# ori-drs/gpmp2

Measured on AMD Instinct MI355X. Metric: trajectories/sec, higher is better.
Workload: dtype f64; 1 GPU; WAMFactorGraphExample: 7-DOF WAM, 100 steps x 5 GP-interp, 200^3 SDF (Synth200), 64 random-init restarts per GPU, GN to tolerance; restarts_per_gpu=64, total_restarts=64, total_step=100, obs_check_inter=5, optimizer=GN, parallelism=trajectory-sharded x1

## Files before the change

gpmp2_amd/_capi.py:

```python
from __future__ import annotations

import ctypes as C

import numpy as np

c_double_p = C.POINTER(C.c_double)
c_int_p = C.POINTER(C.c_int)

OPT_GAUSS_NEWTON, OPT_LM, OPT_DOGLEG = 0, 1, 2
SDF_LAYOUT_ZYX, SDF_LAYOUT_GTSAM = 0, 1
MAX_DOF = 10
MAX_SPHERES = 64

STATUS_NAMES = {0: "converged", 1: "max_iter", 2: "rolled_back", 3: "not_spd", 4: "already_optimal"}


class RobotDesc(C.Structure):
    _fields_ = [("kind", C.c_int), ("dof", C.c_int), ("arm_dof", C.c_int),
                ("a", c_double_p), ("alpha", c_double_p), ("d", c_double_p),
                ("theta_bias", c_double_p), ("base_pose", C.c_double * 16),
                ("nr_spheres", C.c_int), ("sphere_link", c_int_p),
                ("sphere_radius", c_double_p), ("sphere_center", c_double_p),
                ("arm2_dof", C.c_int), ("base_pose2", C.c_double * 16), ("base_pose3", C.c_double * 16),
                ("reverse_linact", C.c_int)]


class Settings(C.Structure):
    _fields_ = [("dof", C.c_int), ("total_step", C.c_int), ("total_time", C.c_double),
                ("conf_prior_sigma", C.c_double), ("vel_prior_sigma", C.c_double),
                ("flag_pos_limit", C.c_int), ("flag_vel_limit", C.c_int),
                ("joint_pos_limits_up", c_double_p), ("joint_pos_limits_down", c_double_p),
                ("vel_limits", c_double_p), ("pos_limit_thresh", c_double_p),
                ("vel_limit_thresh", c_double_p), ("pos_limit_sigmas", c_double_p),
                ("vel_limit_sigmas", c_double_p),
                ("epsilon", C.c_double), ("cost_sigma", C.c_double), ("obs_check_inter", C.c_int),
                ("Qc", c_double_p), ("opt_type", C.c_int), ("verbosity", C.c_int),
                ("final_iter_no_increase", C.c_int), ("rel_thresh", C.c_double),
                ("max_iter", C.c_int)]


MAX_WORKSPACE_FACTORS, MAX_SELF_COLLISION_PAIRS = 4, 16
WORKSPACE_POSITION, WORKSPACE_ORIENTATION, WORKSPACE_POSE = 0, 1, 2


class WorkspaceFactor(C.Structure):
    _fields_ = [("mode", C.c_int), ("link", C.c_int), ("first_state", C.c_int), ("last_state", C.c_int),
                ("sigma", C.c_double), ("des_pose", C.c_double * 16)]


class GraphOpts(C.Structure):
    _fields_ = [("obs_skip_first_state", C.c_int), ("vehicle_dynamics_sigma", C.c_double),
                ("lm_lambda_initial", C.c_double), ("lm_lambda_factor", C.c_double),
                ("lm_lambda_upper", C.c_double), ("lm_lambda_lower", C.c_double),
                ("lm_min_model_fidelity", C.c_double), ("dogleg_delta_initial", C.c_double),
                ("abs_error_tol", C.c_double), ("error_tol", C.c_double),
                ("fixed_iterations", C.c_int),
                ("end_conf_prior_off", C.c_int), ("n_workspace", C.c_int),
                ("workspace", WorkspaceFactor * MAX_WORKSPACE_FACTORS),
                ("n_self_collision", C.c_int), ("self_collision_first", C.c_int), ("self_collision_last", C.c_int),
                ("self_collision", (C.c_double * 4) * MAX_SELF_COLLISION_PAIRS)]


class DebugForms(C.Structure):
    _fields_ = [("lin_split", C.c_int), ("no_fused_finish", C.c_int), ("generic_gn", C.c_int), ("wide_dense", C.c_int),
                ("fail_alloc_at", C.c_int)]


def make_debug_forms(forms):
    unknown = set(forms) - {name for name, _ in DebugForms._fields_}
    if unknown:
        raise ValueError(f"unknown plan forms: {sorted(unknown)}")
    return DebugForms(**{k: int(v) for k, v in forms.items()})


class QueueStats(C.Structure):
    _fields_ = [("passes", C.c_int), ("slot_passes", C.c_long), ("busy_slot_passes", C.c_long)]


def declare_queue(lib):
    vp, i, d = C.c_void_p, C.c_int, c_double_p
    ip = c_int_p
    lib.gpmp2mi_plan_optimize_queue.argtypes = [vp, i, d, d, d, d, d, d, ip, d, ip, d]
    lib.gpmp2mi_plan_optimize_queue.restype = i
    lib.gpmp2mi_plan_optimize_queue_dev.argtypes = [vp, i] + [vp] * 11
    lib.gpmp2mi_plan_optimize_queue_dev.restype = i
    lib.gpmp2mi_plan_queue_stats.argtypes = [vp, C.POINTER(QueueStats)]
    lib.gpmp2mi_plan_queue_stats.restype = i


MAX_SHARDS = 16


def declare_multi(lib):
    vp, i, d, ip = C.c_void_p, C.c_int, c_double_p, c_int_p
    lp = C.POINTER(C.c_long)
    decl = {
        "gpmp2mi_multi_plan_create": [vp, vp, vp, vp, i, i, ip, vp],
        "gpmp2mi_debug_multi_plan_create": [vp, vp, vp, vp, i, i, ip, vp, i, vp],
        "gpmp2mi_multi_plan_shards": [vp, ip, ip, ip],
        "gpmp2mi_multi_plan_set_problem": [vp, d, d, d, d, d],
        "gpmp2mi_multi_plan_optimize": [vp],
        "gpmp2mi_multi_plan_get_result": [vp, d, ip, d, ip, d],
        "gpmp2mi_multi_plan_get_result_dev": [vp, i, vp, vp, vp, vp, vp],
        "gpmp2mi_multi_plan_optimize_queue": [vp, i, d, d, d, d, d, d, ip, d, ip, d],
        "gpmp2mi_multi_plan_queue_stats": [vp, i, C.POINTER(QueueStats)],
        "gpmp2mi_debug_replica_counts": [lp, lp],
        "gpmp2mi_debug_current_device": [i, ip],
    }
    for name, args in decl.items():
        getattr(lib, name).argtypes = args
        getattr(lib, name).restype = i
    lib.gpmp2mi_multi_plan_destroy.argtypes = [vp]
    lib.gpmp2mi_multi_plan_destroy.restype = None


def declare_score(lib):
    vp, i, d, ip, f = C.c_void_p, C.c_int, c_double_p, c_int_p, C.c_double
    decl = {
        "gpmp2mi_score_traj": [vp, vp, f, i, i, i, d, d, d, d, ip, ip],
        "gpmp2mi_score_traj_dev": [vp, vp, f, i, i, i] + [vp] * 7,
        "gpmp2mi_select_best": [i, d, ip, d, ip, f, i, ip, ip],
        "gpmp2mi_select_best_dev": [i, vp, vp, vp, vp, f, i, vp, vp, vp],
        "gpmp2mi_plan_score": [vp, i, d, d, d, ip, ip],
        "gpmp2mi_plan_score_dev": [vp, i] + [vp] * 6,
        "gpmp2mi_plan_select": [vp, i, f, i, ip, ip, d, d],
        "gpmp2mi_plan_select_dev": [vp, i, f, i] + [vp] * 5,
        "gpmp2mi_multi_plan_score": [vp, i, d, d, d, ip, ip],
        "gpmp2mi_multi_plan_select": [vp, i, f, i, ip, ip, d, d],
    }
    for name, args in decl.items():
        getattr(lib, name).argtypes = args
        getattr(lib, name).restype = i


def dptr(a):
    if a is None:
        return None
    assert a.dtype == np.float64 and a.flags["C_CONTIGUOUS"], "need contiguous float64"
    return a.ctypes.data_as(c_double_p)


def iptr(a):
    if a is None:
        return None
    assert a.dtype == np.int32 and a.flags["C_CONTIGUOUS"], "need contiguous int32"
    return a.ctypes.data_as(c_int_p)


# ... 94 lines not shown
```

gpmp2_amd/csrc/assembler.h:

```cpp
#pragma once
#include "device_math.h"
#include "plan.h"
#include "tiles.h"

namespace g2 {

#ifdef G2_STAMPS
#define G2_BSTAMP(k) do { if (i == 1 && lane == 0 && row0 == 0 && col0 == 0 && pb.iters[b] == G2_STAMP_ITER) pb.stamps[(size_t)b * 64 + 24 + (k)] = __builtin_amdgcn_s_memtime(); } while (0)
#else
#define G2_BSTAMP(k) do {} while (0)
#endif

constexpr int GP_EXTRA_LIE = 18;

template <int D, bool LIE>
struct Assembler {
  static constexpr int n = 2 * D, NG = D * (D + 1) / 2, RECP = NG + D + 1;
  static constexpr int GPN = n + 1 + GP_EXTRA_LIE;
  static constexpr int CQ = 24;
  static constexpr int PT_EXTRA_LIE = 36;
  static constexpr int RECMAX = RECP + PT_EXTRA_LIE;

  struct Slot {
    double* base;
// ... 365 lines not shown
              dk[k] = fma(cq[4 + wq[k]], Gn, dk[k]);
              if (want_c) hrk[k] = fma(cq[8 + wq[k]], Gn, hrk[k]);
            }
          }
        }
      }
#pragma unroll
      for (int k = 0; k < 4; k++) {
        dk[k] = valid[k] ? dk[k] : 0.0;
        hrk[k] = valid[k] ? hrk[k] : 0.0;
        hlk[k] = valid[k] ? hlk[k] : 0.0;
      }
    } else {
    v4d xdp = {0.0, 0.0, 0.0, 0.0}, xl = xdp, xdn = xdp, xr = xdp;
    {
      Tile Qt[KT][KT], EL[KT], ER[KT];
#pragma unroll
      for (int ra = 0; ra < KT; ra++)
#pragma unroll
        for (int rb = 0; rb < KT; rb++) Qt[rb][ra] = qc_tile(rb, ra);
      if (has_prev) {
#pragma unroll
        for (int ra = 0; ra < KT; ra++) { EL[ra] = gp_tile(J3i, 1.0, ra, row0); ER[ra] = gp_tile(J3i, 1.0, ra, col0); }
        congruence(Qt, EL, ER, xdp);
        if (want_c) {
#pragma unroll
          for (int ra = 0; ra < KT; ra++) ER[ra] = gp_tile(J1i, -1.0, ra, col0);
          congruence(Qt, EL, ER, xl);
        }
      }
      if (has_next) {
#pragma unroll
        for (int ra = 0; ra < KT; ra++) { EL[ra] = gp_tile(J1n, -1.0, ra, row0); ER[ra] = gp_tile(J1n, -1.0, ra, col0); }
        congruence(Qt, EL, ER, xdn);
        if (want_c) {
#pragma unroll
          for (int ra = 0; ra < KT; ra++) ER[ra] = gp_tile(J3n, 1.0, ra, col0);
          congruence(Qt, EL, ER, xr);
        }
      }
    }
    const double cAxv = -(dt * w0 + w1), cAvv = dt * dt * w0 + 2.0 * dt * w1 + w3, cOvv = -(dt * w1 + w3);
#pragma unroll
    for (int k = 0; k < 4; k++) {
      if (!valid[k]) continue;
      const int ar = a_row[k];
      double d = (ar ? (ac ? w3 : w1) : (ac ? w1 : w0)) * xdp[k] + (ar ? (ac ? cAvv : cAxv) : (ac ? cAxv : w0)) * xdn[k];
      const double hl = (ar ? (ac ? cOvv : w1) : (ac ? cAxv : w0)) * xl[k];
      const double hr = (ar ? (ac ? cOvv : cAxv) : (ac ? w1 : w0)) * xr[k];
      if (!ar && !ac) d += si.pt(I)[tri[k]];
      dk[k] = d;
      hrk[k] = hr;
      hlk[k] = hl;
    }
    lie_interp(si, sn, has_prev, has_next, want_c, dk, hrk, hlk);
    }
    G2_BSTAMP(3);
    for (int e = 0; e < nxp; e++) {
      const size_t xe = (size_t)b * XP_MAX + e;
      if (pb.xp_state[xe] != i) continue;
#pragma unroll
      for (int k = 0; k < 4; k++) {
        if (!valid[k] || a_row[k] != ac || (ac && !pb.xp_has_vel[xe]) || (g + 4 * k) == c) continue;
        dk[k] += pb.xp_info[(xe * 2 + ac) * D * D + (size_t)k_row[k] * D + kc];
      }
    }
    double err_acc = o_ee;
    if (lane <= I && (lane == I || has_prev)) err_acc += si.pt(lane)[NG + D];
    if (lane == 63 && has_prev) err_acc += si.gpr()[n];
#pragma unroll
    for (int k = 0; k < 4; k++) {
      const int rho = g + 4 * k, src = rho - row0;
      const double dsh = __shfl(o_dd, src, 64), gsh = __shfl(o_gg, src, 64);
      double v = dk[k];
      if (rho < n && c == rho) v += dsh;
      if (rho < n && c == rhscol) v = -gsh;
      S.r[k] = v;
      Cr.r[k] = hrk[k];
      Cl.r[k] = hlk[k];
    }
    G2_BSTAMP(4);
    return err_acc;
  }
};

}
```

gpmp2_amd/csrc/cr_kernels.hip:

```cpp
#include "assembler.h"
#include "dispatch.h"
#include "plan_device.h"

namespace g2 {

#ifdef G2_STAMPS
#define G2_STAMP(k)                                                          \
  do {                                                                       \
    if (tid == 0 && (k) < 64 && g2_son) pb.stamps[(size_t)b * 64 + (k)] = __builtin_amdgcn_s_memtime(); \
  } while (0)
#define G2_STAMP_DECL const bool g2_son = pb.iters[b] == G2_STAMP_ITER
#else
#define G2_STAMP(k) do {} while (0)
#define G2_STAMP_DECL do {} while (0)
#endif
#ifdef G2_TSTAMPS
#define G2_TSTAMP(q)                                                                                     \
  do {                                                                                                   \
    if (w == 0 && lane == 0 && idx == 0 && g2_son && (h == 4 || h == 8 || h == 16)) \
      pb.stamps[((size_t)gridDim.x + b) * 64 + (h == 4 ? 0 : h == 8 ? 8 : 16) + (q)] = __builtin_amdgcn_s_memtime(); \
  } while (0)
#else
#define G2_TSTAMP(q) do {} while (0)
#endif
#ifdef G2_STAMPS
#define G2_ASTAMP(k) do { if (i == 1 && lane == 0 && pb.iters[b] == G2_STAMP_ITER) pb.stamps[(size_t)b * 64 + 32 + (k)] = __builtin_amdgcn_s_memtime(); \
                          if (i == 2 && lane == 0 && pb.iters[b] == G2_STAMP_ITER) pb.stamps[(size_t)b * 64 + 40 + (k)] = __builtin_amdgcn_s_memtime(); } while (0)
#else
#define G2_ASTAMP(k) do {} while (0)
#endif

template <int n>
__device__ __forceinline__ void schur_sub(Tile& S, const Tile& A, int lane) {
  const int c = lane & 15, g = lane >> 4;
  const Tile T = tile_atb(A, A);
#pragma unroll
  for (int k = 0; k < 4; k++)
    if ((g + 4 * k) < n && (c < n || c == RHSCOL)) S.r[k] -= T.r[k];
}
constexpr unsigned long long schur_mask(int n, int k) {
  unsigned long long m = 0;
  for (int g = 0; g < 4; g++)
    for (int c = 0; c < 16; c++)
      if (g + 4 * k < n && (c < n || c == RHSCOL)) m |= 1ull << (16 * g + c);
  return m;
}
template <unsigned long long M>
__device__ __forceinline__ double keep_lanes(double x) {
  int lo = __double2loint(x), hi = __double2hiint(x);
  const unsigned long long m = M;
  asm("v_cndmask_b32_e64 %0, 0, %0, %2\n\tv_cndmask_b32_e64 %1, 0, %1, %2" : "+v"(lo), "+v"(hi) : "s"(m));
  return __hiloint2double(hi, lo);
}
template <int n>
__device__ __forceinline__ void schur_keep(Tile& T) {
  T.r[0] = keep_lanes<schur_mask(n, 0)>(T.r[0]);
  T.r[1] = keep_lanes<schur_mask(n, 1)>(T.r[1]);
  T.r[2] = keep_lanes<schur_mask(n, 2)>(T.r[2]);
  T.r[3] = keep_lanes<schur_mask(n, 3)>(T.r[3]);
}
template <int n>
__device__ __forceinline__ Tile schur_prod(const Tile& A, int lane) {
  Tile T = tile_atb(A, A);
  schur_keep<n>(T);
  return T;
}
template <int n>
__device__ __forceinline__ Tile coupling(const Tile& A, const Tile& B, int lane) {
  const int c = lane & 15, g = lane >> 4;
  Tile T = tile_atb(A, B);
#pragma unroll
  for (int k = 0; k < 4; k++) T.r[k] = ((g + 4 * k) < n && c < n) ? -T.r[k] : 0.0;
  return T;
}

constexpr int ASM_WAVES = 4;
#ifndef G2_ASM_MINW
#define G2_ASM_MINW 5
#endif
template <int D, bool LIE>
__global__ __launch_bounds__(64 * ASM_WAVES, LIE ? 2 : G2_ASM_MINW) void k_assemble(const PlanParams* __restrict__ pp, PlanBuffers pb,
                                                              const double* __restrict__ traj, int bufsel,
                                                              double* __restrict__ tiles,
                                                              const int* __restrict__ active) {
  constexpr int n = 2 * D;
  using Asm = Assembler<D, LIE>;
  const PlanParams& P = *pp;
  const int N = P.N;
  const int groups = (N + ASM_WAVES) / ASM_WAVES;
  const int b = blockIdx.x / groups, q = blockIdx.x - b * groups;
  if (active && !active[b]) return;
  if (P.opt_type == GPMP2MI_OPT_DOGLEG && active && pb.phase[b] != 0) return;
  const int wv = threadIdx.x >> 6, lane = threadIdx.x & 63, c = lane & 15, g = lane >> 4;
  const int i = ASM_WAVES * q + wv;
  const bool live = i <= N;
  const int ic = live ? i : N;
  extern __shared__ __attribute__((aligned(16))) double asm_smem[];
  const int slotd = Asm::slot_doubles(P.I, P.RECS, P.GPS);
  double* xch = asm_smem + (size_t)(ASM_WAVES + 1) * slotd;
  double* xs0 = (slotd >= TILE_DBL) ? asm_smem : xch + 4 * TILE_DBL;
  const double* rec = rec_of(pb, pb.which[b], bufsel);
  const double* gpu = gpu_of(pb, pb.which[b], bufsel);
  Asm as(P, pb, rec, gpu, b, lane);
  G2_ASTAMP(0);
  const typename Asm::Slot slot0 = as.make_slot(asm_smem, wv), slot1 = as.make_slot(asm_smem, wv + 1);
  as.stage2(i, slot0, slot1, wv == ASM_WAVES - 1 ? 2 : 1);
  __syncthreads();
  G2_ASTAMP(1);
  const bool odd = (i & 1) != 0;
  const bool fuse2 = N >= 2;
  const bool lvl2 = fuse2 && wv == 2 && live;
  Tile S, Cl, Cr;
  double err_acc = as.build_tiles(ic, slot0, slot1, traj + ((size_t)b * (N + 1) + ic) * n, S, Cl, Cr,
                                  odd || P.opt_type == GPMP2MI_OPT_DOGLEG);
  G2_ASTAMP(2);
  if (live) {
    err_acc = wave_sum(err_acc);
    if (lane == 0) pb.epart[(size_t)b * P.Npad + i] = 0.5 * err_acc;
    if (c == RHSCOL) {
#pragma unroll
      for (int k = 0; k < 4; k++) pb.gvec[((size_t)b * (N + 1) + i) * 16 + g + 4 * k] = -S.r[k];
    }
    if (P.opt_type == GPMP2MI_OPT_DOGLEG) {
      double* ht = pb.htiles + ((size_t)b * (N + 1) + i) * 2 * TILE_DBL;
      tile_store(ht, S, lane);
      tile_store(ht + TILE_DBL, Cr, lane);
    }
    if (P.opt_type == GPMP2MI_OPT_LM) {
      const double lam = pb.lambda[b];
#pragma unroll
      for (int k = 0; k < 4; k++)
        if (g + 4 * k == c && c < n) S.r[k] += lam;
    }
    if (!odd) {
      if (!fuse2) tile_store_rows<n>(tiles + ((size_t)b * (N + 1) + i) * TILE_DBL, S, lane);
      else if (wv == 0) tile_store(xs0, S, lane);
    } else {
      Tile V;
      G2_ASTAMP(3);
      const bool ok = tile_eliminate_cv<n>(S, Cl, Cr, V, lane);
      G2_ASTAMP(4);
      double* f = pb.fac + ((size_t)b * (N + 1) + i) * 3 * TILE_DBL;
      tile_store_rows<n>(f, Cl, lane);
      tile_store_rows<n>(f + TILE_DBL, Cr, lane);
      tile_store_transposed<n>(f + 2 * TILE_DBL, V, lane);
      if (fuse2) {
        double* x = xch + (size_t)(wv >> 1) * 2 * TILE_DBL;
        tile_store(x, Cl, lane);
        tile_store(x + TILE_DBL, Cr, lane);
      }
      if (!ok && lane == 0) pb.notspd[b] = 1;
      G2_ASTAMP(5);
    }
  }
  if (!fuse2) return;
  __syncthreads();
  G2_ASTAMP(6);
  if (wv != 2) return;
  const int j0 = ASM_WAVES * q;
  const bool next = j0 + 4 <= N;
  Tile Sp = tile_load(xs0, lane);
  Tile A1 = tile_zero(), R = tile_zero();
  if (j0 + 1 <= N) {
    const Tile Wl1 = tile_load(xch, lane);
    A1 = tile_atb(Wl1, Wl1);
  }
  if (next && j0 + 3 <= N) {
    const Tile Wr3 = tile_load(xch + 3 * TILE_DBL, lane);
    R = tile_atb(Wr3, Wr3);
  }
  if (live) {
    const int j = i;
    const Tile Wr_m = tile_load(xch + TILE_DBL, lane);
    schur_sub<n>(S, Wr_m, lane);
    const Tile Wl_m = tile_load(xch, lane);
    Tile C2l = coupling<n>(Wr_m, Wl_m, lane);
    Tile C2r = tile_zero();
    if (j + 1 <= N) {
      const Tile Wl_p = tile_load(xch + 2 * TILE_DBL, lane);
      schur_sub<n>(S, Wl_p, lane);
      if (j + 2 <= N) {
        const Tile Wr_p = tile_load(xch + 3 * TILE_DBL, lane);
        C2r = coupling<n>(Wl_p, Wr_p, lane);
      }
    }
    Tile V;
    const bool ok = tile_eliminate_cv<n>(S, C2l, C2r, V, lane);
    double* f = pb.fac + ((size_t)b * (N + 1) + j) * 3 * TILE_DBL;
    tile_store_rows<n>(f, C2l, lane);
    tile_store_rows<n>(f + TILE_DBL, C2r, lane);
    tile_store_transposed<n>(f + 2 * TILE_DBL, V, lane);
    if (!ok && lane == 0) pb.notspd[b] = 1;
    const Tile A2 = tile_atb(C2l, C2l);
#pragma unroll
    for (int k = 0; k < 4; k++) A1.r[k] += A2.r[k];
    if (next) {
      const Tile B2 = tile_atb(C2r, C2r);
#pragma unroll
      for (int k = 0; k < 4; k++) R.r[k] += B2.r[k];
      const Tile K = (q & 1) ? coupling<n>(C2l, C2r, lane) : coupling<n>(C2r, C2l, lane);
      tile_store_rows<n>(pb.coup + ((size_t)b * groups + q) * TILE_DBL, K, lane);
    }
    G2_ASTAMP(7);
  }
  schur_keep<n>(A1);
  schur_keep<n>(R);
#pragma unroll
  for (int k = 0; k < 4; k++) Sp.r[k] -= A1.r[k];
  tile_store_rows<n>(tiles + ((size_t)b * (N + 1) + j0) * TILE_DBL, Sp, lane);
  if (next) tile_store_rows<n>(pb.pend + ((size_t)b * groups + q) * TILE_DBL, R, lane);
}

int launch_assemble(const PlanParams& hp, const PlanBuffers& pb, const double* traj, int bufsel,
                    const int* active, hipStream_t st) {
  const dim3 grid(hp.B * ((hp.N + ASM_WAVES) / ASM_WAVES)), block(64 * ASM_WAVES);
  const size_t slotd = (size_t)(hp.I + 1) * hp.RECS + hp.GPS + 24 * hp.I;
  const size_t shmem = ((ASM_WAVES + 1) * slotd + (slotd >= TILE_DBL ? 4 : 5) * TILE_DBL) * sizeof(double);
  return launch_for_dof(TILE_DOFS, hp.D, [&](auto d) {
    constexpr int D = decltype(d)::value;
    if (hp.lie) k_assemble<D, true><<<grid, block, shmem, st>>>(pb.params, pb, traj, bufsel, pb.tiles, active);
    else k_assemble<D, false><<<grid, block, shmem, st>>>(pb.params, pb, traj, bufsel, pb.tiles, active);
  });
}

constexpr int FIN_BLOCKS = 8;
#ifndef G2_CR_WAVES
#define G2_CR_WAVES 16
#endif
constexpr int CR_WAVES = G2_CR_WAVES;



template <int n>
__device__ __forceinline__ bool cr_forward(const PlanBuffers& pb, int b, int N, int tid) {
  const int w = __builtin_amdgcn_readfirstlane(tid >> 6), lane = tid & 63, c = lane & 15, g = lane >> 4;
  double* tiles = pb.tiles + (size_t)b * (N + 1) * TILE_DBL;
  double* fac = pb.fac + (size_t)b * (N + 1) * 3 * TILE_DBL;
  bool ok = true;
  G2_STAMP_DECL;
  int hfinal = 1;
  while (hfinal <= N) hfinal <<= 1;
  const int h0 = (N >= 2) ? 4 : 2;
  const bool defer4 = (h0 == 4) && (hfinal >= 8);
  for (int h = h0; h <= hfinal; h <<= 1) {
    const bool final = (h == hfinal);
    const int hh = h >> 1;
    const int countE = final ? 1 : ((N / h) + 1) / 2;
    const int countU = (final || (defer4 && h == 4)) ? 0 : (N / (2 * h)) + 1;
    for (int idx = w; idx < countE + countU; idx += CR_WAVES) {
      const bool elim = idx < countE;
      const int j = elim ? (final ? 0 : h * (2 * idx + 1)) : 2 * h * (idx - countE);
      const bool first = h0 == 4 && (h == 4 || (defer4 && h == 8));
      const bool ready = h0 == 4 && h == 4;
      const int jm = j - hh, jp = j + hh, qj = j >> 2;
      const bool em = jm >= 0, ep = jp <= N;
      const bool cm = em && elim && !final, cp = ep && elim && !final && j + h <= N;
      auto facp = [&](int blk, int which) { return fac + ((size_t)blk * 3 + which) * TILE_DBL; };
      const int groups = (N + 4) / 4;
      const double* pend = pb.pend + (size_t)b * groups * TILE_DBL;
      const double* coup = pb.coup + (size_t)b * groups * TILE_DBL;
      G2_TSTAMP(0);
      Tile S = tile_load_rows<n>(tiles + (size_t)j * TILE_DBL, lane);
      Tile Pd = tile_zero();
      Tile Wr_m = tile_zero(), Wl_m = tile_zero(), Wl_p = tile_zero(), Wr_p = tile_zero();
      Tile Cl = tile_zero(), Cr = tile_zero();
      if (first && qj >= 1) Pd = tile_load_rows<n>(pend + (size_t)(qj - 1) * TILE_DBL, lane);
      if (ready) {
        if (cm) Cl = tile_load_rows<n>(coup + (size_t)(qj - 1) * TILE_DBL, lane);
        if (cp) Cr = tile_load_rows<n>(coup + (size_t)qj * TILE_DBL, lane);
      } else {
        if (em) Wr_m = tile_load_rows<n>(facp(jm, 1), lane);
        if (cm) Wl_m = tile_load_rows<n>(facp(jm, 0), lane);
        if (ep) Wl_p = tile_load_rows<n>(facp(jp, 0), lane);
        if (cp) Wr_p = tile_load_rows<n>(facp(jp, 1), lane);
      }
#ifdef G2_TSTAMPS
      asm volatile("s_waitcnt vmcnt(0)" ::: "memory");
#endif
      G2_TSTAMP(1);
#pragma unroll
      for (int k = 0; k < 4; k++) S.r[k] -= Pd.r[k];
      if (!ready) {
        if (em) schur_sub<n>(S, Wr_m, lane);
        if (cm) Cl = coupling<n>(Wr_m, Wl_m, lane);
        if (ep) schur_sub<n>(S, Wl_p, lane);
        if (cp) Cr = coupling<n>(Wl_p, Wr_p, lane);
      }
      if (!elim) {
        tile_store_rows<n>(tiles + (size_t)j * TILE_DBL, S, lane);
        continue;
      }
#ifdef G2_TSTAMPS
      asm volatile("" : "+v"(S.r[0]), "+v"(Cl.r[0]), "+v"(Cr.r[0]));
#endif
      G2_TSTAMP(2);
      Tile V;
      ok = tile_eliminate_cv<n>(S, Cl, Cr, V, lane) && ok;
#ifdef G2_TSTAMPS
      asm volatile("" : "+v"(V.r[0]), "+v"(Cl.r[0]), "+v"(Cr.r[0]));
#endif
      G2_TSTAMP(3);
      double* f = fac + (size_t)j * 3 * TILE_DBL;
      tile_store_rows<n>(f, Cl, lane);
// ... 463 lines not shown
```

gpmp2_amd/csrc/host/host.h:

```cpp
#pragma once
#include <algorithm>
#include <atomic>
#include <memory>
#include <mutex>
#include <string>
#include <vector>

#include "../common.h"
#include "../../../include/gpmp2mi_debug.h"
#include "../launch.h"
#include "../plan.h"

namespace g2 {
const std::string& last_error();

inline int dev_malloc(void** p, size_t bytes, int no_device = GPMP2MI_ERR_ALLOC) {
  const hipError_t e = hipMalloc(p, bytes);
  if (e == hipSuccess) return GPMP2MI_OK;
  *p = nullptr;
  set_error(std::string("hipMalloc: ") + hipGetErrorString(e));
  return (e == hipErrorNoDevice) ? no_device : GPMP2MI_ERR_ALLOC;
}

template <class T>
// ... 38 lines not shown

struct gpmp2mi_robot {
  g2::RobotDev h;
  g2::RobotDev* d = nullptr;
  int device = -1;
  bool replica = false;
  mutable std::mutex score_mu;
  mutable void* score_ws = nullptr;
  mutable size_t score_ws_bytes = 0;
  ~gpmp2mi_robot() {
    if (d) (void)hipFree(d);
    if (score_ws) (void)hipFree(score_ws);
    if (replica) g2::g_robot_replicas.fetch_sub(1);
  }
};
struct gpmp2mi_sdf {
  g2::SdfDev h;
  double* plain = nullptr;
  double* cells = nullptr;
  int device = -1;
  bool replica = false;
  ~gpmp2mi_sdf() {
    if (plain) (void)hipFree(plain);
    if (cells) (void)hipFree(cells);
    if (replica) g2::g_sdf_replicas.fetch_sub(1);
  }
};

namespace g2 {
int sdf_alloc(int dim, const double origin[3], double cell, int nx, int ny, int nz, std::unique_ptr<gpmp2mi_sdf>& s);

struct KernelTimer {
  bool enabled = false;
  struct Rec {
    const char* name;
    hipEvent_t ev;
  };
  std::vector<Rec> recs;
  std::vector<std::string> names;
  std::vector<double> ms;
  std::vector<int> launches;
  std::vector<const char*> cnames;
  std::vector<hipEvent_t> pool;
  size_t pool_used = 0;
  hipEvent_t get() {
    if (pool_used == pool.size()) {
      hipEvent_t e;
      (void)hipEventCreateWithFlags(&e, hipEventDisableSystemFence);
      pool.push_back(e);
    }
    return pool[pool_used++];
  }
  void begin(const char* name, hipStream_t st) {
    if (!enabled) return;
    Rec r{name, get()};
    (void)hipEventRecord(r.ev, st);
    recs.push_back(r);
  }
  void close(hipStream_t st) { begin(nullptr, st); }
  void reset() {
    recs.clear();
    pool_used = 0;
    names.clear();
    ms.clear();
    launches.clear();
  }
  void collect();
  ~KernelTimer() {
    for (auto e : pool) (void)hipEventDestroy(e);
  }
};

struct FlagBuf {
  int* host = nullptr;
  int* dev = nullptr;
  int cap = 0;
  int device = -1;
};
int flags_acquire(int need, FlagBuf* out);
void flags_release(const FlagBuf& f);

struct PlanForms {
  int wide = 0, split_back = 0, wide_h0 = 2, lin_split = 1, fuse_finish = 0, spart_groups = 0;
  bool dense = false;
  bool generic_gn = false;
  bool gn_fast(bool update) const { return !wide && (update || !generic_gn); }
  bool finish_trial(int opt) const { return split_back && opt != GPMP2MI_OPT_DOGLEG && !fuse_finish; }
  bool trial_lin_steps(int opt) const { return fuse_finish && opt != GPMP2MI_OPT_DOGLEG; }
};
}

struct gpmp2mi_plan {
  const gpmp2mi_robot* robot = nullptr;
  const gpmp2mi_sdf* sdf = nullptr;
  g2::PlanParams hp;
  g2::PlanForms forms;
  g2::PlanBuffers pb;
  std::vector<void*> allocs;
  std::vector<size_t> alloc_bytes;
  char* arena_cur = nullptr;
  size_t arena_left = 0;
  int alloc_calls = 0;
  int fail_alloc_at = 0;
  int device = -1;
  g2::FlagBuf flagbuf;
  int* h_flags = nullptr;
  g2::KernelTimer timer;
  int n_active_len = 0;
  std::vector<int> h_xp_n;
  std::vector<char> goal_removed;
  g2::PlanExtras ex;
  bool has_extras = false;
  bool problem_set = false;
  bool optimized = false;
  std::vector<hipStream_t> dirty_streams;
  bool null_stream_dirty = false;
  bool poisoned = false;
  void* qws = nullptr;
  size_t qws_bytes = 0;
  g2::FlagBuf qflags;
  gpmp2mi_queue_stats qstats{};
  bool queue_ran = false;
  void* score_ws = nullptr;
  size_t score_ws_bytes = 0;
  size_t tsz() const { return (size_t)hp.B * (hp.N + 1) * hp.n; }
  void mark_dirty(hipStream_t st) {
    if (!st) { null_stream_dirty = true; return; }
    if (std::find(dirty_streams.begin(), dirty_streams.end(), st) == dirty_streams.end()) dirty_streams.push_back(st);
  }
  void mark_clean(hipStream_t st) {
    if (!st) { null_stream_dirty = false; return; }
    dirty_streams.erase(std::remove(dirty_streams.begin(), dirty_streams.end(), st), dirty_streams.end());
  }
  int close_copies(hipMemcpyKind kind, hipStream_t st) {
    mark_dirty(st);
    if (kind == hipMemcpyDeviceToDevice) return GPMP2MI_OK;
    G2_HIP(hipStreamSynchronize(st));
    mark_clean(st);
    return GPMP2MI_OK;
  }
  void drain() {
    if (poisoned) return;
    for (hipStream_t st : dirty_streams) (void)hipStreamSynchronize(st);
    dirty_streams.clear();
    if (null_stream_dirty) (void)hipStreamSynchronize(nullptr);
    null_stream_dirty = false;
  }
  ~gpmp2mi_plan();
};

#define G2_PLAN_LIVE(p)                         \
  G2_CHECK(!(p)->poisoned, GPMP2MI_ERR_TIMEOUT, \
           "this plan timed out earlier and may still have a hung kernel in its stream: destroy it and create a new one")
#define G2_MULTI_LIVE(m)                                                                                            \
  do {                                                                                                              \
    G2_CHECK(m, GPMP2MI_ERR_INVALID, "null multi plan");                                                            \
    G2_CHECK(!(m)->poisoned, GPMP2MI_ERR_TIMEOUT,                                                                   \
             "a shard of this multi plan timed out earlier and may still have a hung kernel: destroy it and create a new one"); \
  } while (0)

namespace g2 {
struct DeviceGuard {
  int dev = -1;
  DeviceGuard() { if (hipGetDevice(&dev) != hipSuccess) dev = -1; }
  ~DeviceGuard() { if (dev >= 0) (void)hipSetDevice(dev); }
};
// ... 41 lines not shown
```

gpmp2_amd/csrc/host/plan_create.hip:

```cpp
#include <cstring>
#include <mutex>

#include "host.h"

namespace g2 {
static std::mutex g_flag_mu;
static std::vector<FlagBuf> g_flag_pool;
static std::atomic<long> g_live_chunks{0}, g_live_flagbufs{0}, g_leaked_plans{0};
int flags_acquire(int need, FlagBuf* out) {
  {
    std::lock_guard<std::mutex> lk(g_flag_mu);
    int cur = 0;
    (void)hipGetDevice(&cur);
    for (size_t k = 0; k < g_flag_pool.size(); k++)
      if (g_flag_pool[k].cap >= need && g_flag_pool[k].device == cur) {
        *out = g_flag_pool[k];
        g_flag_pool.erase(g_flag_pool.begin() + k);
        g_live_flagbufs.fetch_add(1);
        return GPMP2MI_OK;
      }
  }
  FlagBuf f;
  (void)hipGetDevice(&f.device);
  f.cap = std::max(need, 1024);
// ... 23 lines not shown
      g_chunk_pool.erase(g_chunk_pool.begin() + k);
      return q;
    }
  return nullptr;
}
static void chunk_release(void* q, int device) {
  {
    std::lock_guard<std::mutex> lk(g_flag_mu);
    if (g_chunk_pool.size() < 8) {
      g_chunk_pool.push_back({q, device});
      return;
    }
  }
  (void)hipFree(q);
}
}

using namespace g2;

gpmp2mi_plan::~gpmp2mi_plan() {
  if (poisoned) {
    g_leaked_plans.fetch_add(1);
    return;
  }
  drain();
  for (size_t k = 0; k < allocs.size(); k++) {
    g_live_chunks.fetch_sub(1);
    if (alloc_bytes[k] == ARENA_CHUNK) chunk_release(allocs[k], device);
    else (void)hipFree(allocs[k]);
  }
  flags_release(flagbuf);
  if (qws) (void)hipFree(qws);
  if (score_ws) (void)hipFree(score_ws);
  flags_release(qflags);
}

template <class T>
static int plan_alloc(gpmp2mi_plan* p, T** ptr, size_t count) {
  constexpr size_t ALIGN = 256, CHUNK = ARENA_CHUNK;
  const size_t bytes = (std::max<size_t>(count, 1) * sizeof(T) + ALIGN - 1) / ALIGN * ALIGN;
  if (++p->alloc_calls == p->fail_alloc_at) {
    set_error("hipMalloc: injected failure (gpmp2mi_debug_forms::fail_alloc_at)");
    return GPMP2MI_ERR_ALLOC;
  }
  if (bytes > p->arena_left) {
    const size_t chunk = std::max(bytes, CHUNK);
    void* q = (chunk == CHUNK) ? chunk_acquire() : nullptr;
    if (!q) G2_TRY(dev_malloc(&q, chunk));
    p->allocs.push_back(q);
    p->alloc_bytes.push_back(chunk);
    g_live_chunks.fetch_add(1);
    p->arena_cur = (char*)q;
    p->arena_left = chunk;
    p->null_stream_dirty = true;
    G2_HIP(hipMemsetAsync(q, 0, chunk, nullptr));
  }
  *ptr = (T*)p->arena_cur;
  p->arena_cur += bytes;
  p->arena_left -= bytes;
  return GPMP2MI_OK;
}

static int choose_forms(const RobotDev& h, const gpmp2mi_settings& s, int B, const gpmp2mi_debug_forms* force,
                        PlanForms* out) {
  const gpmp2mi_debug_forms f = force ? *force : gpmp2mi_debug_forms{};
  const int D = h.dof, N = s.total_step, I = s.obs_check_inter;
  const bool fixed_arm = h.kind == GPMP2MI_ROBOT_ARM;
  G2_CHECK(f.lin_split == 0 || f.lin_split == 1 || (fixed_arm && (f.lin_split == 2 || f.lin_split == 4)), GPMP2MI_ERR_UNSUPPORTED,
           "forced lin_split: 1, or 2 / 4 on a fixed-base arm");
  G2_CHECK(f.lin_split != 4 || I >= 2, GPMP2MI_ERR_UNSUPPORTED, "forced lin_split 4: needs obs_check_inter >= 2");
  PlanForms F;
  F.wide = 2 * D > 15;
  G2_CHECK(!f.wide_dense || F.wide, GPMP2MI_ERR_UNSUPPORTED, "forced wide_dense: the plan has no wide blocks (dof < 8)");
  F.dense = D > 11 || f.wide_dense;
  F.split_back = !F.dense && N >= 16;
  while (F.wide && F.wide_h0 < 8 && 4 * F.wide_h0 <= N) F.wide_h0 *= 2;
  const bool four = B <= 256 || s.opt_type != GPMP2MI_OPT_DOGLEG;
  F.lin_split = (fixed_arm && h.nr_spheres >= 2) ? (four ? 4 : 2) : 1;
  if (F.lin_split == 4 && I < 2) F.lin_split = 2;
  if (f.lin_split) F.lin_split = f.lin_split;
  F.fuse_finish = F.lin_split == 4 && F.split_back && !F.wide && !f.no_fused_finish;
  F.spart_groups = F.fuse_finish ? (1 + N * (I + 1) + 63) / 64 : (N + 8) / 8;
  F.generic_gn = f.generic_gn != 0;
  *out = F;
  return GPMP2MI_OK;
}

static int fill_params(const RobotDev& h, const gpmp2mi_settings* s, const gpmp2mi_graph_opts& o, const PlanForms& F,
                       int B, PlanParams& P) {
  const int D = h.dof;
  std::memset(&P, 0, sizeof(P));
  P.B = B;
  P.N = s->total_step;
  P.I = s->obs_check_inter;
  P.P = 1 + P.N * (P.I + 1);
  P.Ppad = (P.P + 63) / 64 * 64;
  P.D = D;
  P.n = 2 * D;
  P.NG = D * (D + 1) / 2;
  P.REC = P.NG + D + 1 + ((h.base_dof == 3 && P.I > 0) ? 36 : 0);
  P.Npad = (P.N + 1 + 63) / 64 * 64;
  P.lie = h.base_dof == 3 ? 1 : 0;
  P.wide = F.wide; P.split_back = F.split_back; P.spart_groups = F.spart_groups;
  P.wide_h0 = F.wide_h0; P.lin_split = F.lin_split; P.fuse_finish = F.fuse_finish;
  P.GPREC = P.n + 1 + (P.lie ? 18 : 0);
  P.RECS = (P.REC + 1) & ~1;
  P.GPS = (P.GPREC + 1) & ~1;
  P.obs_skip_first = o.obs_skip_first_state;
  P.flag_pos_limit = s->flag_pos_limit;
  P.flag_vel_limit = s->flag_vel_limit;
  P.opt_type = s->opt_type;
  P.max_iter = s->max_iter;
  P.no_increase = s->final_iter_no_increase;
  P.fixed_iters = o.fixed_iterations;
  P.end_conf_prior_off = o.end_conf_prior_off ? 1 : 0;
  P.eps = s->epsilon;
  P.obs_w = 1.0 / (s->cost_sigma * s->cost_sigma);
  P.delta_t = s->total_time / static_cast<double>(s->total_step);
  const double inter_dt = P.delta_t / static_cast<double>(s->obs_check_inter + 1);
  P.conf_prior_w = 1.0 / (s->conf_prior_sigma * s->conf_prior_sigma);
  P.vel_prior_w = 1.0 / (s->vel_prior_sigma * s->vel_prior_sigma);
  P.vdyn_w = o.vehicle_dynamics_sigma > 0 ? 1.0 / (o.vehicle_dynamics_sigma * o.vehicle_dynamics_sigma) : 0.0;
  P.rel_thresh = s->rel_thresh;
  P.abs_tol = o.abs_error_tol;
  P.err_tol = o.error_tol;
  P.lm_lambda0 = o.lm_lambda_initial;
  P.lm_factor = o.lm_lambda_factor;
  P.lm_upper = o.lm_lambda_upper;
  P.lm_lower = o.lm_lambda_lower;
  P.lm_min_fidelity = o.lm_min_model_fidelity;
  P.dl_delta0 = o.dogleg_delta_initial;
  for (int j = 0; j < P.I; j++) {
    P.coef[j] = gp_coef(P.delta_t, inter_dt * static_cast<double>(j + 1));
    const double lam[2] = {P.coef[j].l11, P.coef[j].l12}, psi[2] = {P.coef[j].p11, P.coef[j].p12};
    double* q = P.coefq[j];
    for (int ar = 0; ar < 2; ar++)
      for (int ac = 0; ac < 2; ac++) {
        q[0 + ar * 2 + ac] = psi[ar] * psi[ac];
        q[4 + ar * 2 + ac] = lam[ar] * lam[ac];
        q[8 + ar * 2 + ac] = lam[ar] * psi[ac];
        q[12 + ar * 2 + ac] = psi[ar] * lam[ac];
      }
    q[16] = lam[0]; q[17] = lam[1]; q[18] = psi[0]; q[19] = psi[1];
  }
  gp_winv(P.delta_t, P.Winv);
  std::vector<double> Qc(D * D, 0.0), Qi(D * D, 0.0);
  for (int i = 0; i < D; i++) Qc[i * D + i] = 1.0;
  if (s->Qc) std::copy(s->Qc, s->Qc + D * D, Qc.begin());
  G2_CHECK(invert_small(D, Qc.data(), Qi.data()), GPMP2MI_ERR_INVALID, "Qc is singular");
  std::copy(Qi.begin(), Qi.end(), P.Qc_inv);
  for (int k = 0; k < D; k++) {
    P.pos_lo[k] = s->joint_pos_limits_down ? s->joint_pos_limits_down[k] : -1e6;
    P.pos_hi[k] = s->joint_pos_limits_up ? s->joint_pos_limits_up[k] : 1e6;
    P.pos_th[k] = s->pos_limit_thresh ? s->pos_limit_thresh[k] : 1e-3;
    const double ps = s->pos_limit_sigmas ? s->pos_limit_sigmas[k] : 1e-3;
    P.pos_w[k] = 1.0 / (ps * ps);
    P.vel_lim[k] = s->vel_limits ? s->vel_limits[k] : 1e6;
    P.vel_th[k] = s->vel_limit_thresh ? s->vel_limit_thresh[k] : 1e-3;
    const double vs = s->vel_limit_sigmas ? s->vel_limit_sigmas[k] : 1e-3;
    P.vel_w[k] = 1.0 / (vs * vs);
  }
  {
    const int n = P.n;
    const double dt = P.delta_t;
    auto W = [&](int r, int c) { return P.Winv[(r / D) * 2 + (c / D)] * Qi[(r % D) * D + (c % D)]; };
    auto PtW = [&](int r, int c) { return r < D ? W(r, c) : dt * W(r - D, c) + W(r, c); };
    for (int r = 0; r < n; r++)
      for (int c = 0; c < n; c++) {
        P.KB[r * n + c] = W(r, c);
        P.KO[r * n + c] = -PtW(r, c);
        P.KA[r * n + c] = c < D ? PtW(r, c) : dt * PtW(r, c - D) + PtW(r, c);
      }
  }
  const int cap = std::max(P.fixed_iters, P.max_iter);
  P.max_pass = cap * (P.opt_type == GPMP2MI_OPT_LM ? 6 : P.opt_type == GPMP2MI_OPT_DOGLEG ? 18 : 1) + 3;
  return GPMP2MI_OK;
}

struct ExtrasHost {
  std::vector<double> des, scd, radius;
};
static int check_extras(const RobotDev& h, const gpmp2mi_graph_opts& o, int N, PlanExtras& ex, ExtrasHost& hx) {
  std::memset(&ex, 0, sizeof(ex));
  G2_CHECK(o.n_workspace >= 0 && o.n_workspace <= GPMP2MI_MAX_WORKSPACE_FACTORS, GPMP2MI_ERR_INVALID, "too many workspace factors");
  G2_CHECK(o.n_self_collision >= 0 && o.n_self_collision <= GPMP2MI_MAX_SELF_COLLISION_PAIRS, GPMP2MI_ERR_INVALID,
           "too many self-collision pairs");
  ex.n_ws = o.n_workspace;
// ... 190 lines not shown
```

gpmp2_amd/csrc/plan.h:

```cpp
#pragma once
#include "common.h"

namespace g2 {

constexpr int MAXI = 16;
constexpr int TILE = 16;
constexpr int XP_MAX = GPMP2MI_MAX_STATE_PRIORS;

struct PlanParams {
  int B, N, I, P, Ppad, D, n, NG, REC, Npad, GPREC;
  int RECS, GPS;
  int max_pass;
  int obs_skip_first, flag_pos_limit, flag_vel_limit, opt_type, max_iter, no_increase, fixed_iters,
      lie;
  int lin_split;
  int end_conf_prior_off;
  int wide;
  int split_back;
  int spart_groups;
  int wide_h0;
  int fuse_finish;
  double eps, obs_w, delta_t;
  double conf_prior_w, vel_prior_w;
  double vdyn_w;
  double rel_thresh, abs_tol, err_tol;
  double lm_lambda0, lm_factor, lm_upper, lm_lower, lm_min_fidelity, dl_delta0;
  alignas(16) GpCoef coef[MAXI];
  alignas(16) double coefq[MAXI][24];
  double Winv[4];
  double Qc_inv[MAXD * MAXD];
  double pos_lo[MAXD], pos_hi[MAXD], pos_th[MAXD], pos_w[MAXD];
  double vel_lim[MAXD], vel_th[MAXD], vel_w[MAXD];
  double KA[4 * MAXD * MAXD], KB[4 * MAXD * MAXD], KO[4 * MAXD * MAXD];
};

struct PlanExtras {
  int n_ws, n_sc, sc_first, sc_last;
  int ws_mode[GPMP2MI_MAX_WORKSPACE_FACTORS], ws_link[GPMP2MI_MAX_WORKSPACE_FACTORS];
  int ws_first[GPMP2MI_MAX_WORKSPACE_FACTORS], ws_last[GPMP2MI_MAX_WORKSPACE_FACTORS];
  double ws_w[GPMP2MI_MAX_WORKSPACE_FACTORS];
  double sc_w[GPMP2MI_MAX_SELF_COLLISION_PAIRS];
  double* des;
  double* sc_data;
  double* radius;
  double* poses;
  double* Jp;
  double* ws_err;
  double* ws_H;
  double* cen;
  double* Jc;
  double* sc_err;
  double* sc_H;
};

struct PlanBuffers {
  PlanParams* params;
  double* start_conf;
  double* start_vel;
  double* end_conf;
  double* end_vel;
  double* cur;
  double* last;
  double* trial;
  double* init;
  double* result;
  double* rec;
  double* rec2;
  double* gpu;
  double* gpu2;
  double* tiles;
  double* fac;
  double* pend;
  double* coup;
  double* delta;
  double* gvec;
  double* htiles;
  double* hgpart;
  double* scal;
  int* xp_n;
  int* xp_state;
  int* xp_has_vel;
  double* xp_target;
  double* xp_info;
  int* goal_on;
  double* wHd;
  double* wHo;
  double* wg;
  double* wWl;
  double* wWr;
  double* wy;
  double* wrb;
  double* wx;
  double* xg;
  int* stepped;
  double* spart;
  int* which;
  double* cur_err;
  double* prev_err;
  double* last_err;
  double* final_err;
  double* lambda;
  double* trace;
  int* iters;
  int* status;
// ... 81 lines not shown
```

include/gpmp2mi_debug.h:

```cpp
#ifndef GPMP2MI_DEBUG_H
#define GPMP2MI_DEBUG_H

#include "gpmp2mi.h"

#ifdef __cplusplus
extern "C" {
#endif

typedef struct gpmp2mi_debug_forms {
  int lin_split;
  int no_fused_finish;
  int generic_gn;
  int wide_dense;
  int fail_alloc_at;
} gpmp2mi_debug_forms;
int gpmp2mi_debug_plan_create(const gpmp2mi_robot* robot, const gpmp2mi_sdf* sdf,
                              const gpmp2mi_settings* setting, const gpmp2mi_graph_opts* opts ,
                              int B, const gpmp2mi_debug_forms* forms , gpmp2mi_plan** out);
int gpmp2mi_debug_multi_plan_create(const gpmp2mi_robot* robot, const gpmp2mi_sdf* sdf,
                                    const gpmp2mi_settings* setting, const gpmp2mi_graph_opts* opts , int B,
                                    int nshards, const int* devices, const gpmp2mi_debug_forms* forms ,
                                    int replicate_all, gpmp2mi_multi_plan** out);
int gpmp2mi_debug_replica_counts(long* robots, long* sdfs);
int gpmp2mi_debug_current_device(int set_to, int* current);

int gpmp2mi_plan_debug_stamps(gpmp2mi_plan* p, int b, unsigned long long* out64);
int gpmp2mi_plan_debug_scalars(gpmp2mi_plan* p, int b, double* out17);
int gpmp2mi_debug_wait_flag(const int* flag, int timeout_ms, int* value);
int gpmp2mi_debug_resource_counts(long* live_chunks, long* pooled_chunks, long* live_flagbufs, long* pooled_flagbufs,
                                  long* leaked_plans);
int gpmp2mi_debug_stall_begin(void* stream, int max_ms, void** token);
int gpmp2mi_debug_stream_create(void** stream);
int gpmp2mi_debug_stream_destroy(void* stream);
int gpmp2mi_debug_stall_release(void* token);
int gpmp2mi_debug_device_alloc(size_t bytes, int fill_byte, void** out);
int gpmp2mi_debug_device_read(void* dst_host, const void* src_dev, size_t bytes);
int gpmp2mi_debug_device_write(void* dst_dev, const void* src_host, size_t bytes);
int gpmp2mi_debug_device_free(void* p);
int gpmp2mi_debug_crosslane(const double* in64, double* out512);
int gpmp2mi_plan_debug_read(gpmp2mi_plan* p, int which, double* out, long count);

#ifdef __cplusplus
}
#endif
#endif
```

Baseline: 94950 trajectories/sec.

## Split coupling-tile build across waves in assemble kernel for vector-space robots

Adds a split-build path to k_assemble, on by default for non-Lie, non-dogleg, non-wide plans. Odd waves no longer build both coupling tiles and run the combined elimination. Instead the coupling tiles are computed cooperatively by paired waves into shared memory, and each odd wave eliminates only its diagonal tile into an inverse V and then forms Cl and Cr as V^T times the shared tiles. The aim is to balance work across the four waves and shorten the odd waves' critical path, at the cost of an extra __syncthreads, more shared-memory traffic and an extra template instantiation.

```diff
diff --git a/gpmp2_amd/_capi.py b/gpmp2_amd/_capi.py
--- a/gpmp2_amd/_capi.py
+++ b/gpmp2_amd/_capi.py
@@ -63,7 +63,7 @@
 
 class DebugForms(C.Structure):
     _fields_ = [("lin_split", C.c_int), ("no_fused_finish", C.c_int), ("generic_gn", C.c_int), ("wide_dense", C.c_int),
-                ("fail_alloc_at", C.c_int)]
+                ("fail_alloc_at", C.c_int), ("no_split_build", C.c_int)]
 
 
 def make_debug_forms(forms):
diff --git a/gpmp2_amd/csrc/assembler.h b/gpmp2_amd/csrc/assembler.h
--- a/gpmp2_amd/csrc/assembler.h
+++ b/gpmp2_amd/csrc/assembler.h
@@ -471,6 +471,38 @@
     G2_BSTAMP(4);
     return err_acc;
   }
+
+  __device__ __forceinline__ double diag_tile(int i, const Slot& si, const Slot& sn, const double* z, Tile& S) const {
+    Tile Cl, Cr;
+    return build_tiles(i, si, sn, z, S, Cl, Cr, false);
+  }
+  __device__ __forceinline__ Tile coupling_tile(bool left, bool on, const Slot& s) const {
+    static_assert(!LIE, "the coupling tiles of Pose2 robots depend on both states: build_tiles");
+    const int cc_ = min(c, n - 1);
+    const double f = on ? 1.0 : 0.0;
+    const int q0 = left ? 12 : 8;
+    int wq[4];
+    double h[4];
+#pragma unroll
+    for (int k = 0; k < 4; k++) {
+      const int rr_ = min(g + 4 * k, n - 1);
+      wq[k] = q0 + a_row[k] * 2 + a_col;
+      h[k] = f * P.KO[left ? cc_ * n + rr_ : rr_ * n + cc_];
+    }
+    if (on) {
+#pragma unroll 1
+      for (int jj = 0; jj < P.I; jj++) {
+        const double* cq = s.coef(jj);
+        const double* pt_ = s.pt(jj);
+#pragma unroll
+        for (int k = 0; k < 4; k++) h[k] = fma(cq[wq[k]], pt_[tri[k]], h[k]);
+      }
+    }
+    Tile T;
+#pragma unroll
+    for (int k = 0; k < 4; k++) T.r[k] = valid[k] ? h[k] : 0.0;
+    return T;
+  }
 };
 
 }
diff --git a/gpmp2_amd/csrc/cr_kernels.hip b/gpmp2_amd/csrc/cr_kernels.hip
--- a/gpmp2_amd/csrc/cr_kernels.hip
+++ b/gpmp2_amd/csrc/cr_kernels.hip
@@ -75,10 +75,14 @@
 }
 
 constexpr int ASM_WAVES = 4;
+#ifndef G2_ASM_SPLIT_DIV
+#define G2_ASM_SPLIT_DIV 'a'
+#endif
+constexpr char ASM_SPLIT_DIV = G2_ASM_SPLIT_DIV;
 #ifndef G2_ASM_MINW
 #define G2_ASM_MINW 5
 #endif
-template <int D, bool LIE>
+template <int D, bool LIE, bool SPLIT = false>
 __global__ __launch_bounds__(64 * ASM_WAVES, LIE ? 2 : G2_ASM_MINW) void k_assemble(const PlanParams* __restrict__ pp, PlanBuffers pb,
                                                               const double* __restrict__ traj, int bufsel,
                                                               double* __restrict__ tiles,
@@ -110,9 +114,13 @@
   const bool odd = (i & 1) != 0;
   const bool fuse2 = N >= 2;
   const bool lvl2 = fuse2 && wv == 2 && live;
-  Tile S, Cl, Cr;
+  static_assert(!(SPLIT && LIE), "the split build is for vector-space robots");
+  constexpr bool split = SPLIT;
+  Tile S, Cl, Cr, V;
+  bool ok = true;
+  double* const xw = xch + (size_t)(wv >> 1) * 2 * TILE_DBL;
   double err_acc = as.build_tiles(ic, slot0, slot1, traj + ((size_t)b * (N + 1) + ic) * n, S, Cl, Cr,
-                                  odd || P.opt_type == GPMP2MI_OPT_DOGLEG);
+                                  !split && (odd || P.opt_type == GPMP2MI_OPT_DOGLEG));
   G2_ASTAMP(2);
   if (live) {
     err_acc = wave_sum(err_acc);
@@ -121,7 +129,7 @@
 #pragma unroll
       for (int k = 0; k < 4; k++) pb.gvec[((size_t)b * (N + 1) + i) * 16 + g + 4 * k] = -S.r[k];
     }
-    if (P.opt_type == GPMP2MI_OPT_DOGLEG) {
+    if (!split && P.opt_type == GPMP2MI_OPT_DOGLEG) {
       double* ht = pb.htiles + ((size_t)b * (N + 1) + i) * 2 * TILE_DBL;
       tile_store(ht, S, lane);
       tile_store(ht + TILE_DBL, Cr, lane);
@@ -135,19 +143,48 @@
     if (!odd) {
       if (!fuse2) tile_store_rows<n>(tiles + ((size_t)b * (N + 1) + i) * TILE_DBL, S, lane);
       else if (wv == 0) tile_store(xs0, S, lane);
-    } else {
-      Tile V;
+    } else if (split) {
+      if (c == RHSCOL) {
+#pragma unroll
+        for (int k = 0; k < 4; k++) xw[k * 64 + lane] = xw[TILE_DBL + k * 64 + lane] = S.r[k];
+      }
+    }
+  }
+  if constexpr (split) {
+    const int nt = ASM_SPLIT_DIV == 'a' ? ((wv & 1) ? 0 : 2) : 1;
+#pragma unroll
+    for (int u = 0; u < 2; u++) {
+      const int t = wv + u, j = ASM_WAVES * q + 1 + (t & 2);
+      if (u >= nt || j > N) continue;
+      const bool left = !(t & 1);
+      const Tile T = as.coupling_tile(left, left || j < N, as.make_slot(asm_smem, t + 1));
+      if (c != RHSCOL) tile_store(xch + (size_t)t * TILE_DBL, T, lane);
+    }
+    if (live && odd) {
+#pragma unroll
+      for (int k = 0; k < 4; k++) V.r[k] = (g + 4 * k == c && c < n) ? 1.0 : 0.0;
       G2_ASTAMP(3);
-      const bool ok = tile_eliminate_cv<n>(S, Cl, Cr, V, lane);
+      ok = tile_eliminate_col<n>(S, V, lane);
+    }
+    __syncthreads();
+  }
+  if (live) {
+    if (odd) {
+      if constexpr (split) {
+        Cl = tile_atb(V, tile_load(xw, lane));
+        Cr = tile_atb(V, tile_load(xw + TILE_DBL, lane));
+      } else {
+        G2_ASTAMP(3);
+        ok = tile_eliminate_cv<n>(S, Cl, Cr, V, lane);
+      }
       G2_ASTAMP(4);
       double* f = pb.fac + ((size_t)b * (N + 1) + i) * 3 * TILE_DBL;
       tile_store_rows<n>(f, Cl, lane);
       tile_store_rows<n>(f + TILE_DBL, Cr, lane);
       tile_store_transposed<n>(f + 2 * TILE_DBL, V, lane);
       if (fuse2) {
-        double* x = xch + (size_t)(wv >> 1) * 2 * TILE_DBL;
-        tile_store(x, Cl, lane);
-        tile_store(x + TILE_DBL, Cr, lane);
+        tile_store(xw, Cl, lane);
+        tile_store(xw + TILE_DBL, Cr, lane);
       }
       if (!ok && lane == 0) pb.notspd[b] = 1;
       G2_ASTAMP(5);
@@ -219,6 +256,7 @@
   return launch_for_dof(TILE_DOFS, hp.D, [&](auto d) {
     constexpr int D = decltype(d)::value;
     if (hp.lie) k_assemble<D, true><<<grid, block, shmem, st>>>(pb.params, pb, traj, bufsel, pb.tiles, active);
+    else if (hp.split_build) k_assemble<D, false, true><<<grid, block, shmem, st>>>(pb.params, pb, traj, bufsel, pb.tiles, active);
     else k_assemble<D, false><<<grid, block, shmem, st>>>(pb.params, pb, traj, bufsel, pb.tiles, active);
   });
 }
diff --git a/gpmp2_amd/csrc/host/host.h b/gpmp2_amd/csrc/host/host.h
--- a/gpmp2_amd/csrc/host/host.h
+++ b/gpmp2_amd/csrc/host/host.h
@@ -144,6 +144,7 @@
 
 struct PlanForms {
   int wide = 0, split_back = 0, wide_h0 = 2, lin_split = 1, fuse_finish = 0, spart_groups = 0;
+  int split_build = 0;
   bool dense = false;
   bool generic_gn = false;
   bool gn_fast(bool update) const { return !wide && (update || !generic_gn); }
diff --git a/gpmp2_amd/csrc/host/plan_create.hip b/gpmp2_amd/csrc/host/plan_create.hip
--- a/gpmp2_amd/csrc/host/plan_create.hip
+++ b/gpmp2_amd/csrc/host/plan_create.hip
@@ -129,6 +129,7 @@
   F.fuse_finish = F.lin_split == 4 && F.split_back && !F.wide && !f.no_fused_finish;
   F.spart_groups = F.fuse_finish ? (1 + N * (I + 1) + 63) / 64 : (N + 8) / 8;
   F.generic_gn = f.generic_gn != 0;
+  F.split_build = !F.wide && h.base_dof != 3 && s.opt_type != GPMP2MI_OPT_DOGLEG && !f.no_split_build;
   *out = F;
   return GPMP2MI_OK;
 }
@@ -150,6 +151,7 @@
   P.lie = h.base_dof == 3 ? 1 : 0;
   P.wide = F.wide; P.split_back = F.split_back; P.spart_groups = F.spart_groups;
   P.wide_h0 = F.wide_h0; P.lin_split = F.lin_split; P.fuse_finish = F.fuse_finish;
+  P.split_build = F.split_build;
   P.GPREC = P.n + 1 + (P.lie ? 18 : 0);
   P.RECS = (P.REC + 1) & ~1;
   P.GPS = (P.GPREC + 1) & ~1;
diff --git a/gpmp2_amd/csrc/plan.h b/gpmp2_amd/csrc/plan.h
--- a/gpmp2_amd/csrc/plan.h
+++ b/gpmp2_amd/csrc/plan.h
@@ -20,6 +20,7 @@
   int spart_groups;
   int wide_h0;
   int fuse_finish;
+  int split_build;
   double eps, obs_w, delta_t;
   double conf_prior_w, vel_prior_w;
   double vdyn_w;
diff --git a/include/gpmp2mi_debug.h b/include/gpmp2mi_debug.h
--- a/include/gpmp2mi_debug.h
+++ b/include/gpmp2mi_debug.h
@@ -13,6 +13,7 @@
   int generic_gn;
   int wide_dense;
   int fail_alloc_at;
+  int no_split_build;
 } gpmp2mi_debug_forms;
 int gpmp2mi_debug_plan_create(const gpmp2mi_robot* robot, const gpmp2mi_sdf* sdf,
                               const gpmp2mi_settings* setting, const gpmp2mi_graph_opts* opts ,
```

Result: faster. 95920 trajectories/sec, median of 3 (+1.0%).
